# Hansard-T/FHE-Linformer

Measured on AMD Instinct MI355X. Metric: encrypted Linformer-d128 forward ms/sample, lower is better.
Workload: dtype u64

## Files before the change

fhe-linformer_amd/csrc/context.cpp:

```cpp
#include "context.h"
#include <hip/hip_runtime.h>
#include <algorithm>
#include <cstdio>
#include <cstdlib>
#include <cstring>
#include <sys/random.h>
#include <time.h>
#include <cxxabi.h>
#include <dlfcn.h>
#include <execinfo.h>

namespace fhelin {

void hip_check(hipError_t e, const char* what) {
    if (e != hipSuccess) throw Error(FHELIN_ERR_HIP, std::string(what) + ": " + hipGetErrorString(e));
}

void* DevicePool::raw_malloc(size_t bytes) {
    if (backend_.malloc_fn) return backend_.malloc_fn(bytes);
    void* p = nullptr;
    if (hipMalloc(&p, bytes) != hipSuccess) {
        (void)hipGetLastError();
        return nullptr;
    }
    return p;
}
void DevicePool::raw_free(void* p) {
    if (backend_.free_fn) backend_.free_fn(p);
    else (void)hipFree(p);
}
DevicePool::~DevicePool() {
    for (auto& ln : lane_) {
        for (auto& pk : ln.parked)
            for (int k = 0; k < pk.n_ev; ++k) (void)hipEventDestroy(pk.ev[k]);
        for (auto& sl : ln.slabs)
            if (sl.base) raw_free(sl.base);
    }
    for (hipEvent_t e : spare_events_) (void)hipEventDestroy(e);
}
size_t DevicePool::slabs() const {
    size_t n = 0;
    for (const auto& ln : lane_)
        for (const auto& sl : ln.slabs) n += sl.base != nullptr;
    return n;
}
size_t DevicePool::free_ranges() const {
    size_t n = 0;
    for (const auto& ln : lane_) n += ln.by_size.size();
    return n;
}
void DevicePool::erase_size_entry(Lane& ln, int slab, size_t off, size_t len) {
    auto r = ln.by_size.equal_range(len);
    for (auto it = r.first; it != r.second; ++it)
        if (it->second.first == slab && it->second.second == off) {
            ln.by_size.erase(it);
            return;
        }
    throw Error(FHELIN_ERR_INTERNAL, "DevicePool: free list out of step");
}
void DevicePool::insert_free(Lane& ln, int slab, size_t off, size_t len) {
    Slab& sl = ln.slabs[slab];
    auto nxt = sl.free_at.lower_bound(off);
    if (nxt != sl.free_at.begin()) {
        auto prv = std::prev(nxt);
        if (prv->first + prv->second == off) {
            off = prv->first;
            len += prv->second;
            erase_size_entry(ln, slab, prv->first, prv->second);
            sl.free_at.erase(prv);
        }
    }
    if (nxt != sl.free_at.end() && off + len == nxt->first) {
        len += nxt->second;
        erase_size_entry(ln, slab, nxt->first, nxt->second);
        sl.free_at.erase(nxt);
    }
    sl.free_at[off] = len;
    ln.by_size.emplace(len, std::make_pair(slab, off));
}
bool DevicePool::grow(Lane& ln, size_t bytes) {
    size_t want = std::max(bytes, std::min(SLAB_MAX, std::max(SLAB_MIN, reserved_)));
    want = (want + (size_t(2) << 20) - 1) & ~((size_t(2) << 20) - 1);
    timespec t0, t1;
    clock_gettime(CLOCK_MONOTONIC, &t0);
    void* p = raw_malloc(want);
// ... 149 lines not shown
        for (int i = 0; i < 8; ++i) p.seed_bytes[i] = (uint8_t)(p.seed >> (8 * i));
    } else {
        size_t got = 0;
        while (got < sizeof p.seed_bytes) {
            const ssize_t n = getrandom(p.seed_bytes + got, sizeof p.seed_bytes - got, 0);
            if (n <= 0) throw Error(FHELIN_ERR_INTERNAL, "getrandom failed: no entropy for key generation");
            got += (size_t)n;
        }
    }
    p.have_seed_bytes = true;
}

static Params resolve_params(Params p) {
    resolve_seed(p);
    if (p.n_p < 0 && p.n_q >= 1 && p.dnum >= 1 && p.special_bits >= 1) {
        const int a = (p.n_q + p.dnum - 1) / p.dnum;
        const int first = p.first_bits + (std::min(a, p.n_q) - 1) * p.scale_bits;
        const int other = p.n_q > a ? std::min(a, p.n_q - a) * p.scale_bits : 0;
        p.n_p = (std::max(first, other) + p.special_bits - 1) / p.special_bits;
    }
    return p;
}

Context::Context(const Params& p_in) : prm(resolve_params(p_in)) {
    const Params& p = prm;
    if (p.log_n < 12 || p.log_n > 17) throw Error(FHELIN_ERR_ARG, "log_n must be in [12,17]");
    if (p.n_q < 1 || p.n_q > 64 || p.n_p < 0 || p.n_p > 16) throw Error(FHELIN_ERR_ARG, "bad limb counts");
    if (p.dnum < 1) throw Error(FHELIN_ERR_ARG, "dnum must be >= 1");
    if (p.first_bits > 60 || p.scale_bits > 60 || p.special_bits > 60) throw Error(FHELIN_ERR_ARG, "primes must be <= 60 bits");
    if (p.first_bits < 20 || p.scale_bits < 20 || (p.n_p > 0 && p.special_bits < 20)) throw Error(FHELIN_ERR_ARG, "primes must be >= 20 bits");
    if (p.log_slots < 1 || p.log_slots > p.log_n - 1) throw Error(FHELIN_ERR_ARG, "log_slots out of range");
    N = 1 << p.log_n;
    L = p.n_q - 1;
    K = p.n_p;
    alpha = (p.n_q + p.dnum - 1) / p.dnum;
    if (alpha > 16) throw Error(FHELIN_ERR_ARG, "digit size > 16 limbs not supported");
    if ((p.n_q + alpha - 1) / alpha > 16) throw Error(FHELIN_ERR_ARG, "more than 16 key-switching digits not supported");
    try {
        chain = make_prime_chain(p.log_n, p.n_q, p.first_bits, p.scale_bits, p.n_p, p.special_bits);
    } catch (const std::exception& e) {
        throw Error(FHELIN_ERR_ARG, std::string("prime chain: ") + e.what());
    }
    moduli = chain.q;
    moduli.insert(moduli.end(), chain.p.begin(), chain.p.end());
    for (u64 q : moduli) {
        barrett.push_back(h_barrett(q));
        tw.push_back(make_twiddles(q, p.log_n));
    }
    sf_real.assign(p.n_q + 1, 0.0L);
    sf_real[0] = (long double)chain.q[L];
    for (int k = 0; k < L; ++k) sf_real[k + 1] = sf_real[k] * sf_real[k] / (long double)chain.q[L - k];

    if (p.device < 0) return;

    int ndev = 0;
    if (hipGetDeviceCount(&ndev) != hipSuccess || ndev <= 0)
        throw Error(FHELIN_ERR_NO_DEVICE, "no HIP device visible: the fhe-linformer_amd engine has no CPU fallback");
    if (p.device >= ndev) throw Error(FHELIN_ERR_ARG, "device index out of range");
    hip_check(hipSetDevice(p.device), "hipSetDevice");
    hip_check(hipStreamCreateWithFlags(&stream, hipStreamNonBlocking), "hipStreamCreate");
    main_stream = stream;
    own_stream = true;
    {
        int want = 2;
        if (const char* e = std::getenv("FHELIN_LANES")) want = std::atoi(e);
        n_lanes = std::max(0, std::min(want, DevicePool::MAX_LANES - 1));
        for (int k = 1; k <= n_lanes; ++k) {
            hip_check(hipStreamCreateWithFlags(&lane_stream[k], hipStreamNonBlocking), "hipStreamCreate(lane)");
            hip_check(hipEventCreateWithFlags(&lane_event[k], hipEventDisableTiming), "hipEventCreate(lane)");
        }
        hip_check(hipEventCreateWithFlags(&fork_event, hipEventDisableTiming), "hipEventCreate(fork)");
        pool.lane_stream[0] = main_stream;
        for (int k = 1; k <= n_lanes; ++k) pool.lane_stream[k] = lane_stream[k];
        pool.have_streams = true;
        if (const char* e = std::getenv("FHELIN_ASYNC")) async_lanes = std::atoi(e) != 0;
        if (const char* e = std::getenv("FHELIN_FUSE_MODDOWN")) fuse_moddown = std::atoi(e) != 0;
        if (const char* e = std::getenv("FHELIN_FUSE_FINISH")) fuse_finish = std::atoi(e) != 0;
        if (const char* e = std::getenv("FHELIN_HOST_ENCODE")) host_encode = std::atoi(e) != 0;
        if (const char* e = std::getenv("FHELIN_FUSE_GATHER")) fuse_gather = std::atoi(e) != 0;
        if (const char* e = std::getenv("FHELIN_FUSE_LIFT")) fuse_lift = std::atoi(e) != 0;
        if (const char* e = std::getenv("FHELIN_LDS_DIGITS")) lds_digits = std::atoi(e) != 0;
        if (const char* e = std::getenv("FHELIN_NTT_TRACE")) trace_small_ntt = std::atoi(e);
        if (const char* e = std::getenv("FHELIN_HOST_WAITS")) trace_waits = std::atoi(e) != 0;
    }
    hip_check(hipEventCreate(&ev_start), "hipEventCreate");
    stage_words = (size_t)2 << p.log_n;
    for (int i = 0; i < STAGE_SLOTS; ++i) {
        hip_check(hipHostMalloc(reinterpret_cast<void**>(&stage_buf[i]), stage_words * sizeof(u64), hipHostMallocDefault), "hipHostMalloc(stage)");
        hip_check(hipEventCreateWithFlags(&stage_ev[i], hipEventDisableTiming), "hipEventCreate(stage)");
    }
    hip_check(hipHostMalloc(reinterpret_cast<void**>(&small_buf), (size_t)SMALL_SLOTS * SMALL_WORDS * sizeof(u64), hipHostMallocDefault), "hipHostMalloc(stage, small)");
    for (int i = 0; i < SMALL_SLOTS; ++i) hip_check(hipEventCreateWithFlags(&small_ev[i], hipEventDisableTiming), "hipEventCreate(stage, small)");
    hip_check(hipEventCreate(&ev_stop), "hipEventCreate");
    has_device = true;

    const int nl = (int)moduli.size();
    {
        std::vector<u64> bar(2 * nl), ninv(8 * nl, 0);
        for (int i = 0; i < nl; ++i) {
            bar[2 * i] = barrett[i].r0;
            bar[2 * i + 1] = barrett[i].r1;
            ninv[8 * i] = tw[i].n_inv;
            ninv[8 * i + 1] = tw[i].n_inv_s;
            ninv[8 * i + 2] = tw[i].w1_n_inv;
            ninv[8 * i + 3] = tw[i].w1_n_inv_s;
            int bits = 0;
            while (bits < 64 && (moduli[i] >> bits)) ++bits;
            if (bits >= 12 && bits <= 60) {
                ninv[8 * i + 4] = (u64)(bits - 10);
                ninv[8 * i + 5] = (u64)((((u128)1) << (bits + 22)) / moduli[i]);
            }
        }
        dt.log_n = p.log_n;
        dt.n_limbs = nl;
        dt.moduli = upload_table(moduli);
        dt.barrett = upload_table(bar);
        {
            std::vector<u64> qi(nl);
            for (int i = 0; i < nl; ++i) {
                u64 x = moduli[i];
                for (int it = 0; it < 6; ++it) x *= 2 - moduli[i] * x;
                qi[i] = x;
            }
            dt.qinv = upload_table(qi);
            std::vector<u64> mr(2 * (size_t)nl);
            for (int i = 0; i < nl; ++i) {
                mr[2 * i] = mont_r(moduli[i]);
                mr[2 * i + 1] = h_shoup(mr[2 * i], moduli[i]);
            }
            dt.mont = upload_table(mr);
        }
        dt.ninv = upload_table(ninv);
        std::vector<u64> f((size_t)nl * 2 * N), g((size_t)nl * 2 * N);
        for (int i = 0; i < nl; ++i) {
            std::memcpy(&f[(size_t)i * 2 * N], tw[i].fwd.data(), sizeof(u64) * 2 * N);
            std::memcpy(&g[(size_t)i * 2 * N], tw[i].inv.data(), sizeof(u64) * 2 * N);
        }
        dt.tw_fwd = upload_table(f);
        dt.tw_inv = upload_table(g);
        const size_t tiles = N >> 12;
        const size_t per_limb = tiles * 15 * 256 * 2;
        for (int dir = 0; dir < 2; ++dir) {
            const std::vector<u64>& src = dir ? g : f;
            std::vector<u64> r((size_t)nl * per_limb);
            for (int i = 0; i < nl; ++i)
                for (size_t T = 0; T < tiles; ++T)
                    for (int kb = 0; kb < 4; ++kb)
                        for (int j = 0; j < (8 >> kb); ++j)
                            for (size_t tau = 0; tau < 256; ++tau) {
                                const size_t idx = (N >> (kb + 1)) + ((((T << 8) | tau)) << (3 - kb)) + j;
                                const size_t s_ = (size_t)(8 >> kb) - 1 + j;
                                const size_t o = (size_t)i * per_limb + ((T * 15 + s_) * 256 + tau) * 2;
                                r[o] = src[(size_t)i * 2 * N + 2 * idx];
                                r[o + 1] = src[(size_t)i * 2 * N + 2 * idx + 1];
                            }
            (dir ? dt.tw_rows_inv : dt.tw_rows_fwd) = upload_table(r);
        }
    }
    {
        std::vector<u64> phatinv(2 * std::max(K, 1)), phatmod((size_t)std::max(K, 1) * (L + 1)), pinv(2 * (L + 1));
        for (int j = 0; j < K; ++j) {
            u64 pj = chain.p[j];
            u64 hat = prod_mod(chain.p, j, pj);
            u64 inv = h_invmod(hat, pj);
            phatinv[2 * j] = inv;
            phatinv[2 * j + 1] = h_shoup(inv, pj);
// ... 275 lines not shown
```

fhe-linformer_amd/csrc/context.h:

```cpp
#pragma once
#include <cstdint>
#include <map>
#include <memory>
#include <stdexcept>
#include <string>
#include <unordered_map>
#include <vector>
#include <hip/hip_runtime_api.h>
#include "../../include/fhelin.h"
#include "hostmath.h"
#include "kernels.h"

namespace fhelin {

struct Params {
    int log_n = 16;
    int n_q = 24;
    int first_bits = 55;
    int scale_bits = 52;
    int n_p = 6;
    int special_bits = 60;
    int dnum = 4;
    int log_slots = 14;
    int hamming = 192;
// ... 94 lines not shown
    int L = 0;
    int K = 0;
    int alpha = 0;
    PrimeChain chain;
    std::vector<u64> moduli;
    std::vector<Barrett> barrett;
    std::vector<TwiddleTable> tw;
    std::vector<long double> sf_real;

    bool has_device = false;
    hipStream_t stream = nullptr;
    hipStream_t main_stream = nullptr;
    bool own_stream = false;
    int n_lanes = 0;
    hipStream_t lane_stream[DevicePool::MAX_LANES] = {};
    hipEvent_t lane_event[DevicePool::MAX_LANES] = {};
    hipEvent_t fork_event = nullptr;
    bool async_lanes = true;
    int async_rr = 0;
    u64 lane_seq[DevicePool::MAX_LANES] = {};
    std::vector<std::pair<u64, std::shared_ptr<void>>> lane_hold[DevicePool::MAX_LANES];
    void release_holds(int lane, u64 up_to_seq);
    void fork_lanes();
    void join_lanes();
    struct LaneScope {
        Context& c;
        LaneScope(Context& ctx, int k) : c(ctx) {
            c.stream = c.lane_stream[k];
            c.pool.cur_lane = k;
        }
        ~LaneScope() {
            c.stream = c.main_stream;
            c.pool.cur_lane = 0;
        }
    };
    DevicePool pool;
    DeviceTables dt{};
    std::vector<void*> table_allocs;
    hipEvent_t ev_start = nullptr, ev_stop = nullptr;

    static constexpr int STAGE_SLOTS = 64;
    u64* stage_buf[STAGE_SLOTS] = {};
    hipEvent_t stage_ev[STAGE_SLOTS] = {};
    bool stage_used[STAGE_SLOTS] = {};
    int stage_next = 0;
    size_t stage_words = 0;
    static constexpr int SMALL_SLOTS = 256;
    static constexpr size_t SMALL_WORDS = 8192;
    u64* small_buf = nullptr;
    hipEvent_t small_ev[SMALL_SLOTS] = {};
    bool small_used[SMALL_SLOTS] = {};
    int small_next = 0;
    void upload_async(u64* dst, const u64* src, size_t words);

    const u64* d_phatinv = nullptr;
    const u64* d_phatmod = nullptr;
    const u64* d_pinv = nullptr;
    const u64* d_pmod = nullptr;
    const u64* d_qlinv = nullptr;
    const u64* d_qlmod = nullptr;
    std::vector<LevelTables> lvl;
    std::map<u64, const u32*> automorph_maps;

    explicit Context(const Params& p);
    ~Context();
    Context(const Context&) = delete;
    Context& operator=(const Context&) = delete;

    void require_device() const;
    template <class T> T* dalloc(size_t count) { return static_cast<T*>(pool.alloc(count * sizeof(T))); }
    template <class T> const T* upload_table(const std::vector<T>& v);
    int limb_id_q(int i) const { return i; }
    int limb_id_p(int j) const { return L + 1 + j; }
    int digits_at(int ell) const { return (ell + alpha - 1) / alpha; }
    u64 galois_element(int rot_index) const;
    const u32* automorph_map(u64 galois);
    const u32* automorph_inverse_of(const u32* map);
    std::map<const u32*, const u32*> automorph_inverse;
    bool fuse_finish = true;
    bool fuse_moddown = false;
    bool host_encode = false;
    bool fuse_gather = true;
    bool fuse_lift = true;
    bool lds_digits = true;
    struct FftDev {
        const u32* rot = nullptr;
        const double* ksi = nullptr;
    };
    std::map<int, FftDev> fft_dev;
    void sync();
    void ntt(const LimbBatch& b, bool inverse, int active = -1) {
        stats.limb_ntt += (u64)(active >= 0 ? active : b.nvec);
        if (trace_small_ntt && b.nvec <= trace_small_ntt) note_small_ntt(b.nvec);
        launch_ntt(dt, b, inverse, stream);
    }
    bool trace_waits = false;
    std::map<std::string, std::pair<u64, u64>> wait_sites;
    void note_wait(const char* site, u64 ns) {
        auto& e = wait_sites[site];
        e.first += 1;
        e.second += ns;
    }
    int trace_small_ntt = 0;
    std::map<std::string, std::pair<u64, u64>> small_ntt_sites;
    void note_small_ntt(int nvec);
    void ntt_epilogue(const LimbBatch& b, const NttEpilogue& ep) {
        stats.limb_ntt += (u64)b.nvec;
        if (trace_small_ntt && b.nvec <= trace_small_ntt) note_small_ntt(b.nvec);
        launch_ntt_epilogue(dt, b, ep, stream);
    }
};

}
```

fhe-linformer_amd/csrc/kernels.h:

```cpp
#pragma once
#include <cstddef>
#include <cstdint>
#include <hip/hip_runtime_api.h>
#include "modarith.h"

namespace fhelin {

struct LimbBatch {
    u64* data;
    int nvec;
    const int* limb_tab;
    int limb_first;
    int limb_count;
    const u64* src = nullptr;
    int tab_len = 0;
    int src_group = 0;
    size_t src_group_stride = 0;
    int src_group2 = 0;
    size_t src_group2_stride = 0;
    bool lazy_out = false;
    const u64* lift_qlm = nullptr;
    int lift_limb = -1;
};

struct DeviceTables {
    int log_n;
    int n_limbs;
    const u64* moduli;
    const u64* barrett;
    const u64* qinv;
    const u64* mont;
    const u64* tw_fwd;
    const u64* tw_inv;
    const u64* tw_rows_fwd;
    const u64* tw_rows_inv;
    const u64* ninv;
};

struct NttEpilogue {
    static constexpr int MAX_ROWS = 16;
    const u64* acc = nullptr;
    size_t acc_poly_stride = 0;
    u64* out = nullptr;
    size_t out_stride = 0;
    const u64* w = nullptr;
    int ell = 0;
    const u64* add0 = nullptr;
    const u64* add1 = nullptr;
    const u64* post = nullptr;
    size_t add_stride = 0, post_stride = 0;
    const u32* invmap = nullptr;
    int per_row = 0;
    const u32* invmap_row[MAX_ROWS] = {};
};

void launch_ntt(const DeviceTables& t, const LimbBatch& b, bool inverse, hipStream_t s);
void launch_ntt_epilogue(const DeviceTables& t, const LimbBatch& b, const NttEpilogue& ep, hipStream_t s);


}
```

fhe-linformer_amd/csrc/kernels_ntt.hip:

```cpp
#include <hip/hip_runtime.h>
#include <algorithm>
#include <cstdlib>
#include "kernels.h"

namespace fhelin {

namespace {

struct NttArgs {
    u64* data;
    const u64* src;
    const u64* tw;
    const u64* tw_rows;
    const u64* moduli;
    const u64* ninv;
    const int* limb_tab;
    int tab_len;
    int limb_first;
    int limb_count;
    int log_n;
    int nvec;
    int period;
    int lazy_out;
    int src_group;
    size_t src_group_stride;
    int src_group2;
    size_t src_group2_stride;
    const u64* lift_qlm;
    int lift_limb;
    int vec0;
};

__device__ __forceinline__ size_t src_offset(const NttArgs& a, int vec, int log_n) {
    if (a.src_group > 0) {
        const int g = vec / a.src_group;
        const size_t in = (size_t)(vec % a.src_group) << log_n;
        if (a.src_group2 > 0) return (size_t)(g / a.src_group2) * a.src_group2_stride + (size_t)(g % a.src_group2) * a.src_group_stride + in;
        return (size_t)g * a.src_group_stride + in;
    }
    return (size_t)vec << log_n;
}

constexpr int TILE = 4096;
constexpr int LDS_WORDS = TILE + TILE / 16;

__device__ __forceinline__ int tile_index(int tau, int k, int p) {
    return ((tau >> p) << (p + 4)) | (k << p) | (tau & ((1 << p) - 1));
}
__device__ __forceinline__ int lds_slot(int e) { return e + (e >> 4); }

__device__ __forceinline__ int limb_of(const NttArgs& a, int vec) {
    return a.limb_tab ? a.limb_tab[a.tab_len ? vec % a.tab_len : vec] : a.limb_first + (vec % a.limb_count);
}

typedef u64 u64x2 __attribute__((ext_vector_type(2)));

struct LimbConst {
    u64 q;
    u64 nq;
    u64 q5;
    u32 sh;
    u32 rr;
};

struct RoundTw {
    u64x2 t[15];
};
template <int KB_LO, int KB_HI>
__device__ __forceinline__ void load_round_tw(RoundTw& r, const u64x2* __restrict__ tw, int log_n, int gbase, int hi) {
#pragma unroll
    for (int kb = KB_LO; kb < KB_HI; ++kb) {
        const int m = 1 << (log_n - (gbase + kb) - 1);
        const int tbase = m + (hi << (3 - kb));
#pragma unroll
        for (int j = 0; j < (8 >> kb); ++j) r.t[(8 >> kb) - 1 + j] = tw[tbase + j];
    }
}

__device__ __forceinline__ void load_round_tw_rows(RoundTw& r, const u64x2* __restrict__ trows, int tau) {
#pragma unroll
    for (int s = 0; s < 15; ++s) r.t[s] = trows[s * 256 + tau];
}

template <int KB, bool LAZY>
__device__ __forceinline__ void fwd_stage(u64 (&x)[16], const RoundTw& tw, const LimbConst& c) {
#pragma unroll
    for (int k0 = 0; k0 < 16; ++k0) {
        if (k0 & (1 << KB)) continue;
        const int k1 = k0 | (1 << KB);
        const u64x2 w = tw.t[(8 >> KB) - 1 + (k0 >> (KB + 1))];
        const u64 X = LAZY ? x[k0] : csub_mask(x[k0], c.q5);
#if defined(FHELIN_BFLY15)
        const u64 T = mul_shoup_lazy5(x[k1], w.x, w.y, c.nq);
        x[k0] = X + T;
        x[k1] = X + c.q5 - T;
#else
        const u64 A = mul_shoup_lazy5_add(x[k1], w.x, w.y, c.nq, X);
        x[k0] = A;
        x[k1] = shl1_add(X, c.q5) - A;
#endif
    }
}
template <int KB_LO, int KB_HI, bool LAZY>
__device__ __forceinline__ void fwd_round(u64 (&x)[16], const RoundTw& tw, const LimbConst& c) {
    if constexpr (KB_LO < KB_HI) {
        fwd_stage<KB_HI - 1, LAZY>(x, tw, c);
        fwd_round<KB_LO, KB_HI - 1, LAZY>(x, tw, c);
    }
}

constexpr int lazy_coef(int s, int c0) { return s == 0 ? c0 : 5 << (s - 1); }

template <int KB, bool FINAL, bool LAZY, int S, int C0>
__device__ __forceinline__ void inv_stage(u64 (&x)[16], const RoundTw& tw, const LimbConst& c, const u64* __restrict__ ninv) {
    const u64 B = c.q * (u64)lazy_coef(S, C0);
    if constexpr (FINAL) {
        const u64 ni = ninv[0], nis = ninv[1], wn = ninv[2], wns = ninv[3];
#pragma unroll
        for (int k0 = 0; k0 < 16; ++k0) {
            if (k0 & (1 << KB)) continue;
            const int k1 = k0 | (1 << KB);
            const u64 X = x[k0], Y = x[k1];
            if (LAZY) {
                x[k0] = csub_mask(reduce_lazy_2q(mul_shoup_lazy5(X + Y, ni, nis, c.nq), c.q, c.sh, c.rr), c.q);
                x[k1] = csub_mask(reduce_lazy_2q(mul_shoup_lazy5(X + B - Y, wn, wns, c.nq), c.q, c.sh, c.rr), c.q);
            } else {
                x[k0] = csub_mask(reduce_lazy_2q(mul_shoup_lazy5(X + Y, ni, nis, c.nq), c.q, c.sh, c.rr), c.q);
                x[k1] = csub_mask(reduce_lazy_2q(mul_shoup_lazy5(X + c.q5 - Y, wn, wns, c.nq), c.q, c.sh, c.rr), c.q);
            }
        }
    } else {
#pragma unroll
        for (int k0 = 0; k0 < 16; ++k0) {
            if (k0 & (1 << KB)) continue;
            const int k1 = k0 | (1 << KB);
            const u64x2 w = tw.t[(8 >> KB) - 1 + (k0 >> (KB + 1))];
            const u64 X = x[k0], Y = x[k1];
            if (LAZY) {
                x[k0] = X + Y;
                x[k1] = mul_shoup_lazy5(X + B - Y, w.x, w.y, c.nq);
            } else {
                x[k0] = csub_mask(X + Y, c.q5);
                x[k1] = mul_shoup_lazy5(X + c.q5 - Y, w.x, w.y, c.nq);
            }
        }
    }
}
template <int KB_LO, int KB_HI, bool LAST, bool LAZY, int S0 = 0, int C0 = 1>
__device__ __forceinline__ void inv_round(u64 (&x)[16], const RoundTw& tw, const LimbConst& c, const u64* __restrict__ ninv) {
    if constexpr (KB_LO < KB_HI) {
        inv_stage<KB_LO, (LAST && KB_LO == KB_HI - 1), LAZY, S0, C0>(x, tw, c, ninv);
        inv_round<KB_LO + 1, KB_HI, LAST, LAZY, S0 + 1, C0>(x, tw, c, ninv);
    }
}

__device__ __forceinline__ void exchange(u64 (&x)[16], u64* lds, int tau, int p_from, int p_to, bool sync_first) {
    if (sync_first) __syncthreads();
#pragma unroll
    for (int k = 0; k < 16; ++k) lds[lds_slot(tile_index(tau, k, p_from))] = x[k];
    __syncthreads();
#pragma unroll
    for (int k = 0; k < 16; ++k) x[k] = lds[lds_slot(tile_index(tau, k, p_to))];
}

__device__ __forceinline__ LimbConst limb_const(const NttArgs& a, int limb) {
    LimbConst c;
    c.q = a.moduli[limb];
    c.nq = 0 - c.q;
    c.q5 = 5 * c.q;
    c.sh = (u32)a.ninv[8 * limb + 4];
    c.rr = (u32)a.ninv[8 * limb + 5];
    return c;
}
#if defined(FHELIN_NTT_FORCE_PATH)
template <bool INVERSE> __device__ __forceinline__ bool lazy_prime(u64) { return FHELIN_NTT_FORCE_PATH; }
#else
template <bool INVERSE> __device__ __forceinline__ bool lazy_prime(u64 q) { return q < (1ull << (INVERSE ? 53 : 57)); }
#endif

template <int A, bool INVERSE, bool LAZY, bool LIFT>
__device__ __forceinline__ void cols_body(const NttArgs& a, u64* lds, int vec, int tile, int limb, const LimbConst& c) {
    constexpr int LOGCW = 12 - A;
    constexpr int CW = 1 << LOGCW;
    constexpr int LOGN = A + 8;
    constexpr int NFULL = A / 4;
    constexpr int REM = A % 4;
    const u64x2* tw = reinterpret_cast<const u64x2*>(a.tw) + ((size_t)limb << LOGN);
    u64* base = a.data + ((size_t)vec << LOGN) + tile * CW;
    const u64* sbase = (LIFT ? a.src + ((size_t)(vec / a.limb_count) << LOGN) : a.src + src_offset(a, vec, LOGN)) + tile * CW;
    const int tau = threadIdx.x;
    u64 x[16];

    auto goff = [](int e) { return ((e >> LOGCW) << 8) | (e & (CW - 1)); };

    if (!INVERSE) {
        constexpr int P0 = LOGCW + A - 4;
#pragma unroll
        for (int k = 0; k < 16; ++k) x[k] = sbase[goff(tile_index(tau, k, P0))];
        if constexpr (LIFT) {
            const u64 half = a.moduli[a.lift_limb] >> 1, qlm = a.lift_qlm[limb];
#pragma unroll
            for (int k = 0; k < 16; ++k) {
                const u64 r = csub_mask(x[k], c.q);
                x[k] = x[k] > half ? sub_mod(r, qlm, c.q) : r;
            }
        }
        RoundTw rt, rn;
        load_round_tw<0, 4>(rt, tw, LOGN, 8 + P0 - LOGCW, tau >> P0);
        fwd_round<0, 4, LAZY>(x, rt, c);
        int p_prev = P0;
        if constexpr (NFULL >= 2) {
            constexpr int P1 = LOGCW + A - 8;
            load_round_tw<0, 4>(rn, tw, LOGN, 8 + P1 - LOGCW, tau >> P1);
            exchange(x, lds, tau, p_prev, P1, false);
            fwd_round<0, 4, LAZY>(x, rn, c);
            p_prev = P1;
        }
        if constexpr (REM > 0) {
            constexpr int PR = LOGCW;
            load_round_tw<0, REM>(rt, tw, LOGN, 8, tau >> PR);
            exchange(x, lds, tau, p_prev, PR, NFULL >= 2);
            fwd_round<0, REM, LAZY>(x, rt, c);
            p_prev = PR;
        }
        constexpr int PL = REM > 0 ? LOGCW : (NFULL >= 2 ? LOGCW + A - 8 : P0);
        (void)p_prev;
#pragma unroll
        for (int k = 0; k < 16; ++k) base[goff(tile_index(tau, k, PL))] = x[k];
    } else {
        const u64* ninv = a.ninv + 8 * limb;
        constexpr int P0 = LOGCW;
#pragma unroll
        for (int k = 0; k < 16; ++k) x[k] = sbase[goff(tile_index(tau, k, P0))];
        RoundTw rt, rn;
        load_round_tw<0, 4>(rt, tw, LOGN, 8, tau >> P0);
        inv_round<0, 4, (NFULL == 1 && REM == 0), LAZY, 0, 2>(x, rt, c, ninv);
        int p_prev = P0;
        if constexpr (NFULL >= 2) {
            constexpr int P1 = LOGCW + 4;
            load_round_tw<0, 4>(rn, tw, LOGN, 8 + 4, tau >> P1);
            exchange(x, lds, tau, p_prev, P1, false);
            inv_round<0, 4, (REM == 0), LAZY, 4, 2>(x, rn, c, ninv);
            p_prev = P1;
        }
        if constexpr (REM > 0) {
            constexpr int PR = 8;
            load_round_tw<4 - REM, 4>(rt, tw, LOGN, 8 + PR - LOGCW, tau >> PR);
            exchange(x, lds, tau, p_prev, PR, NFULL >= 2);
            inv_round<4 - REM, 4, true, LAZY, 4 * NFULL, 2>(x, rt, c, ninv);
            p_prev = PR;
        }
        constexpr int PL = REM > 0 ? 8 : (NFULL >= 2 ? LOGCW + 4 : P0);
        (void)p_prev;
#pragma unroll
        for (int k = 0; k < 16; ++k) base[goff(tile_index(tau, k, PL))] = x[k];
    }
}

template <int A, bool INVERSE, bool LIFT = false>
__global__ __launch_bounds__(256) __attribute__((amdgpu_waves_per_eu(LIFT ? 3 : 4))) void ntt_cols_kernel(NttArgs a) {
    constexpr int LOGTILES = A - 4;
    __shared__ u64 lds[LDS_WORDS];
    const int vec = a.vec0 + (blockIdx.x >> LOGTILES);
    const int tile = blockIdx.x & ((1 << LOGTILES) - 1);
    const int limb = limb_of(a, vec);
    if (limb < 0) return;
    const LimbConst c = limb_const(a, limb);
    if (lazy_prime<INVERSE>(c.q))
        cols_body<A, INVERSE, true, LIFT>(a, lds, vec, tile, limb, c);
    else
        cols_body<A, INVERSE, false, LIFT>(a, lds, vec, tile, limb, c);
}

template <bool INVERSE, bool LAZY, bool EPI>
__device__ __forceinline__ void rows_body(const NttArgs& a, u64* lds, int vec, int tile, int limb, const LimbConst& c,
                                          const NttEpilogue* ep) {
    const int log_n = a.log_n;
    const u64x2* tw = reinterpret_cast<const u64x2*>(a.tw) + ((size_t)limb << log_n);
    const u64x2* trows = reinterpret_cast<const u64x2*>(a.tw_rows) + (((size_t)limb << (log_n - 12)) + tile) * (15 * 256);
    u64* base = a.data + ((size_t)vec << log_n) + ((size_t)tile << 12);
    const u64* sbase = a.src + src_offset(a, vec, log_n) + ((size_t)tile << 12);
    const int tau = threadIdx.x;
    u64 x[16];

    if (!INVERSE) {
#pragma unroll
        for (int k = 0; k < 16; ++k) x[k] = sbase[tile_index(tau, k, 4)];
        RoundTw rt, rn;
        load_round_tw<0, 4>(rt, tw, log_n, 4, (tile << 4) | (tau >> 4));
        fwd_round<0, 4, LAZY>(x, rt, c);
        load_round_tw_rows(rn, trows, tau);
        exchange(x, lds, tau, 4, 0, false);
        fwd_round<0, 4, LAZY>(x, rn, c);
        [[maybe_unused]] u64 av[16];
        [[maybe_unused]] int ell = 0, t = 0, poly = 0;
        if constexpr (EPI) {
            ell = ep->ell;
            t = vec % ell;
            poly = vec / ell;
            const u64* acc = ep->acc + (size_t)poly * ep->acc_poly_stride + ((size_t)t << log_n) + ((size_t)tile << 12);
#pragma unroll
            for (int k = 0; k < 16; ++k) av[k] = acc[tile_index(tau, k, 8)];
        }
        if constexpr (EPI) {
#pragma unroll
            for (int k = 0; k < 16; ++k) x[k] = reduce_lazy_2q(x[k], c.q, c.sh, c.rr);
        } else if (!(LAZY && a.lazy_out && c.q < (1ull << 53))) {
#pragma unroll
            for (int k = 0; k < 16; ++k)
                x[k] = csub_mask(reduce_lazy_2q(x[k], c.q, c.sh, c.rr), c.q);
        }
#if defined(FHELIN_ROWS_DIRECT_STORE)
        if constexpr (!EPI) {
#pragma unroll
            for (int k = 0; k < 16; k += 2) {
                u64x2 v;
                v.x = x[k];
                v.y = x[k + 1];
                reinterpret_cast<u64x2*>(base + 16 * tau)[k >> 1] = v;
            }
            return;
        }
#endif
        exchange(x, lds, tau, 0, 8, true);
        if constexpr (EPI) {
            const int bi = poly >> 1, comp = poly & 1;
            const size_t n = (size_t)1 << log_n;
            const u64 w = ep->w[2 * t], ws = ep->w[2 * t + 1];
            const u64 q2 = 2 * c.q;
#pragma unroll
            for (int k = 0; k < 16; ++k) x[k] = mul_shoup(av[k] + q2 - x[k], w, ws, c.q);
            const u64* add = comp == 0 ? ep->add0 : ep->add1;
            if (add) {
                add += (size_t)bi * ep->add_stride + (size_t)t * n + ((size_t)tile << 12);
#pragma unroll
                for (int k = 0; k < 16; ++k) x[k] = add_mod(x[k], add[tile_index(tau, k, 8)], c.q);
            }
            const size_t row_off = (size_t)(comp * ell + t) * n;
            const u64* post = ep->post ? ep->post + (size_t)bi * ep->post_stride + row_off : nullptr;
            u64* out = ep->out + (size_t)bi * ep->out_stride + row_off;
            const u32* im = ep->per_row ? ep->invmap_row[bi] : ep->invmap;
            if (im) {
#pragma unroll
                for (int k = 0; k < 16; ++k) {
                    const size_t j = im[((size_t)tile << 12) + tile_index(tau, k, 8)];
                    u64 r = x[k];
                    if (post) r = add_mod(r, post[j], c.q);
                    out[j] = r;
                }
            } else {
                out += (size_t)tile << 12;
                if (post) {
                    post += (size_t)tile << 12;
#pragma unroll
                    for (int k = 0; k < 16; ++k) x[k] = add_mod(x[k], post[tile_index(tau, k, 8)], c.q);
                }
#pragma unroll
                for (int k = 0; k < 16; ++k) out[tile_index(tau, k, 8)] = x[k];
            }
        } else {
#pragma unroll
            for (int k = 0; k < 16; ++k) base[tile_index(tau, k, 8)] = x[k];
        }
    } else {
#pragma unroll
        for (int k = 0; k < 16; ++k) x[k] = sbase[tile_index(tau, k, 8)];
        RoundTw rt, rn;
        load_round_tw_rows(rt, trows, tau);
        exchange(x, lds, tau, 8, 0, false);
        inv_round<0, 4, false, LAZY, 0, 1>(x, rt, c, nullptr);
        load_round_tw<0, 4>(rn, tw, log_n, 4, (tile << 4) | (tau >> 4));
        exchange(x, lds, tau, 0, 4, true);
        inv_round<0, 4, false, LAZY, 4, 1>(x, rn, c, nullptr);
        if (LAZY) {
#pragma unroll
            for (int k = 0; k < 16; ++k) x[k] = reduce_lazy_2q(x[k], c.q, c.sh, c.rr);
        }
#pragma unroll
        for (int k = 0; k < 16; ++k) base[tile_index(tau, k, 4)] = x[k];
    }
}

template <bool INVERSE, bool EPI = false>
__global__ __launch_bounds__(256) __attribute__((amdgpu_waves_per_eu(4))) void ntt_rows_kernel(NttArgs a, NttEpilogue ep) {
    __shared__ u64 lds[LDS_WORDS];
    const int logtiles = a.log_n - 12;
    int lid = blockIdx.x;
    const int nblk = gridDim.x;
    if ((nblk & 7) == 0) lid = (lid & 7) * (nblk >> 3) + (lid >> 3);
    int vec, tile;
    if (a.period > 0) {
        const int nper = a.nvec / a.period;
        const int rep = lid % nper, r = lid / nper;
        tile = r & ((1 << logtiles) - 1);
        vec = a.vec0 + rep * a.period + (r >> logtiles);
    } else {
        vec = a.vec0 + (lid >> logtiles);
        tile = lid & ((1 << logtiles) - 1);
    }
    const int limb = limb_of(a, vec);
    if (limb < 0) return;
    const LimbConst c = limb_const(a, limb);
    if (lazy_prime<INVERSE>(c.q))
        rows_body<INVERSE, true, EPI>(a, lds, vec, tile, limb, c, &ep);
    else
        rows_body<INVERSE, false, EPI>(a, lds, vec, tile, limb, c, &ep);
}

template <int A>
void launch_cols(const NttArgs& a, bool inverse, int blocks, hipStream_t s) {
    if (inverse)
        hipLaunchKernelGGL((ntt_cols_kernel<A, true>), dim3(blocks), dim3(256), 0, s, a);
    else if (a.lift_qlm)
        hipLaunchKernelGGL((ntt_cols_kernel<A, false, true>), dim3(blocks), dim3(256), 0, s, a);
    else
        hipLaunchKernelGGL((ntt_cols_kernel<A, false>), dim3(blocks), dim3(256), 0, s, a);
}

}

static void launch_ntt_impl(const DeviceTables& t, const LimbBatch& b, bool inverse, const NttEpilogue* ep, hipStream_t s);

void launch_ntt(const DeviceTables& t, const LimbBatch& b, bool inverse, hipStream_t s) { launch_ntt_impl(t, b, inverse, nullptr, s); }
void launch_ntt_epilogue(const DeviceTables& t, const LimbBatch& b, const NttEpilogue& ep, hipStream_t s) {
    launch_ntt_impl(t, b, false, &ep, s);
}

static void launch_ntt_impl(const DeviceTables& t, const LimbBatch& b, bool inverse, const NttEpilogue* ep, hipStream_t s) {
    if (b.nvec <= 0) return;
    NttArgs a;
    a.data = b.data;
    a.src = b.src ? b.src : b.data;
    a.src_group = b.src ? b.src_group : 0;
    a.src_group_stride = b.src_group_stride;
    a.src_group2 = (b.src && b.src_group > 0) ? b.src_group2 : 0;
    a.src_group2_stride = b.src_group2_stride;
    a.lazy_out = (!inverse && b.lazy_out) ? 1 : 0;
    a.lift_qlm = (!inverse && b.src && b.lift_limb >= 0) ? b.lift_qlm : nullptr;
    a.lift_limb = b.lift_limb;
    a.tw = inverse ? t.tw_inv : t.tw_fwd;
    a.tw_rows = inverse ? t.tw_rows_inv : t.tw_rows_fwd;
    a.moduli = t.moduli;
    a.ninv = t.ninv;
    a.limb_tab = b.limb_tab;
    a.tab_len = b.tab_len;
    a.limb_first = b.limb_first;
    a.limb_count = b.limb_count > 0 ? b.limb_count : 1;
    a.log_n = t.log_n;
    a.nvec = b.nvec;
    const int per = b.limb_tab ? b.tab_len : a.limb_count;
    a.period = (per > 0 && per < b.nvec && b.nvec % per == 0) ? per : 0;
    const int A = t.log_n - 8;
    a.vec0 = 0;
    static const int chunk_mb = [] {
        const char* e = std::getenv("FHELIN_NTT_CHUNK_MB");
        return e ? std::atoi(e) : 0;
    }();
    int chunk = b.nvec;
    if (chunk_mb > 0 && !ep) {
        const size_t vec_bytes = (size_t)8 << t.log_n;
        const int want = (int)std::max<size_t>(1, ((size_t)chunk_mb << 20) / vec_bytes);
        if (b.nvec > want + want / 2) {
            const int per = a.period > 0 ? a.period : 1;
            chunk = std::max(per, want / per * per);
        }
    }
    const int nvec_all = b.nvec, period_all = a.period;
    const u64* src_all = a.src;
    const int sg = a.src_group, sg2 = a.src_group2;
    for (int v0 = 0; v0 < nvec_all; v0 += chunk) {
        a.vec0 = v0;
        a.nvec = std::min(chunk, nvec_all - v0);
        a.period = (period_all > 0 && a.nvec % period_all == 0 && a.nvec > period_all) ? period_all : 0;
        a.src = src_all;
        a.src_group = sg;
        a.src_group2 = sg2;
        const int blocks = a.nvec << (t.log_n - 12);
        auto cols = [&]() {
            switch (A) {
                case 4: launch_cols<4>(a, inverse, blocks, s); break;
                case 5: launch_cols<5>(a, inverse, blocks, s); break;
                case 6: launch_cols<6>(a, inverse, blocks, s); break;
                case 7: launch_cols<7>(a, inverse, blocks, s); break;
                case 8: launch_cols<8>(a, inverse, blocks, s); break;
                case 9: launch_cols<9>(a, inverse, blocks, s); break;
                default: break;
            }
        };
        if (!inverse) {
            cols();
            a.src = a.data;
            a.src_group = 0;
            a.src_group2 = 0;
            if (ep)
                hipLaunchKernelGGL((ntt_rows_kernel<false, true>), dim3(blocks), dim3(256), 0, s, a, *ep);
            else
                hipLaunchKernelGGL((ntt_rows_kernel<false, false>), dim3(blocks), dim3(256), 0, s, a, NttEpilogue());
        } else {
            hipLaunchKernelGGL((ntt_rows_kernel<true, false>), dim3(blocks), dim3(256), 0, s, a, NttEpilogue());
            a.src = a.data;
            a.src_group = 0;
            a.src_group2 = 0;
            cols();
        }
    }
}

}
```

Measured before the change: 239.4.

## Add narrow NTT kernels with more threads per tile for small batches

Adds NTT column and row kernel variants that hold 8 (or 4) elements per thread instead of 16, launched with 512 or 1024 threads per 4096-element tile. They are selected when the launch has fewer blocks than a CU-count-based threshold, so small NTT batches can fill the GPU with more threads. The cost is extra LDS exchange rounds and barriers per tile, plus more template instantiations. An environment variable can force the narrow path on or off.

Result: no change. 238.2 (median of 6 runs) (-0.5%).

```diff
diff --git a/fhe-linformer_amd/csrc/context.cpp b/fhe-linformer_amd/csrc/context.cpp
--- a/fhe-linformer_amd/csrc/context.cpp
+++ b/fhe-linformer_amd/csrc/context.cpp
@@ -1,6 +1,7 @@
 #include "context.h"
 #include <hip/hip_runtime.h>
 #include <algorithm>
+#include <climits>
 #include <cstdio>
 #include <cstdlib>
 #include <cstring>
@@ -316,6 +317,17 @@
         if (const char* e = std::getenv("FHELIN_LDS_DIGITS")) lds_digits = std::atoi(e) != 0;
         if (const char* e = std::getenv("FHELIN_NTT_TRACE")) trace_small_ntt = std::atoi(e);
         if (const char* e = std::getenv("FHELIN_HOST_WAITS")) trace_waits = std::atoi(e) != 0;
+        int cus = 0;
+        hip_check(hipDeviceGetAttribute(&cus, hipDeviceAttributeMultiprocessorCount, p.device), "hipDeviceGetAttribute(CUs)");
+        dt.ntt_narrow_below = NTT_NARROW_BLOCKS_PER_CU * std::max(cus, 1);
+        if (const char* e = std::getenv("FHELIN_NTT_NARROW")) {
+            if (!std::strcmp(e, "0"))
+                dt.ntt_narrow_below = 0;
+            else if (!std::strcmp(e, "1"))
+                dt.ntt_narrow_below = INT_MAX;
+            else if (std::strcmp(e, "auto"))
+                throw Error(FHELIN_ERR_ARG, "FHELIN_NTT_NARROW must be auto, 0 or 1");
+        }
     }
     hip_check(hipEventCreate(&ev_start), "hipEventCreate");
     stage_words = (size_t)2 << p.log_n;
diff --git a/fhe-linformer_amd/csrc/context.h b/fhe-linformer_amd/csrc/context.h
--- a/fhe-linformer_amd/csrc/context.h
+++ b/fhe-linformer_amd/csrc/context.h
@@ -200,6 +200,7 @@
     bool host_encode = false;
     bool fuse_gather = true;
     bool fuse_lift = true;
+    static constexpr int NTT_NARROW_BLOCKS_PER_CU = 6;
     bool lds_digits = true;
     struct FftDev {
         const u32* rot = nullptr;
diff --git a/fhe-linformer_amd/csrc/kernels.h b/fhe-linformer_amd/csrc/kernels.h
--- a/fhe-linformer_amd/csrc/kernels.h
+++ b/fhe-linformer_amd/csrc/kernels.h
@@ -35,6 +35,7 @@
     const u64* tw_rows_fwd;
     const u64* tw_rows_inv;
     const u64* ninv;
+    int ntt_narrow_below;
 };
 
 struct NttEpilogue {
diff --git a/fhe-linformer_amd/csrc/kernels_ntt.hip b/fhe-linformer_amd/csrc/kernels_ntt.hip
--- a/fhe-linformer_amd/csrc/kernels_ntt.hip
+++ b/fhe-linformer_amd/csrc/kernels_ntt.hip
@@ -44,9 +44,11 @@
 constexpr int TILE = 4096;
 constexpr int LDS_WORDS = TILE + TILE / 16;
 
+template <int W = 4>
 __device__ __forceinline__ int tile_index(int tau, int k, int p) {
-    return ((tau >> p) << (p + 4)) | (k << p) | (tau & ((1 << p) - 1));
-}
+    return ((tau >> p) << (p + W)) | (k << p) | (tau & ((1 << p) - 1));
+}
+constexpr int log2i(int r) { return r <= 1 ? 0 : 1 + log2i(r / 2); }
 __device__ __forceinline__ int lds_slot(int e) { return e + (e >> 4); }
 
 __device__ __forceinline__ int limb_of(const NttArgs& a, int vec) {
@@ -63,9 +65,11 @@
     u32 rr;
 };
 
-struct RoundTw {
-    u64x2 t[15];
+template <int R>
+struct RoundTwR {
+    u64x2 t[R - 1];
 };
+using RoundTw = RoundTwR<16>;
 template <int KB_LO, int KB_HI>
 __device__ __forceinline__ void load_round_tw(RoundTw& r, const u64x2* __restrict__ tw, int log_n, int gbase, int hi) {
 #pragma unroll
@@ -82,13 +86,13 @@
     for (int s = 0; s < 15; ++s) r.t[s] = trows[s * 256 + tau];
 }
 
-template <int KB, bool LAZY>
-__device__ __forceinline__ void fwd_stage(u64 (&x)[16], const RoundTw& tw, const LimbConst& c) {
-#pragma unroll
-    for (int k0 = 0; k0 < 16; ++k0) {
+template <int KB, bool LAZY, int R>
+__device__ __forceinline__ void fwd_stage(u64 (&x)[R], const RoundTwR<R>& tw, const LimbConst& c) {
+#pragma unroll
+    for (int k0 = 0; k0 < R; ++k0) {
         if (k0 & (1 << KB)) continue;
         const int k1 = k0 | (1 << KB);
-        const u64x2 w = tw.t[(8 >> KB) - 1 + (k0 >> (KB + 1))];
+        const u64x2 w = tw.t[((R / 2) >> KB) - 1 + (k0 >> (KB + 1))];
         const u64 X = LAZY ? x[k0] : csub_mask(x[k0], c.q5);
 #if defined(FHELIN_BFLY15)
         const u64 T = mul_shoup_lazy5(x[k1], w.x, w.y, c.nq);
@@ -101,8 +105,8 @@
 #endif
     }
 }
-template <int KB_LO, int KB_HI, bool LAZY>
-__device__ __forceinline__ void fwd_round(u64 (&x)[16], const RoundTw& tw, const LimbConst& c) {
+template <int KB_LO, int KB_HI, bool LAZY, int R>
+__device__ __forceinline__ void fwd_round(u64 (&x)[R], const RoundTwR<R>& tw, const LimbConst& c) {
     if constexpr (KB_LO < KB_HI) {
         fwd_stage<KB_HI - 1, LAZY>(x, tw, c);
         fwd_round<KB_LO, KB_HI - 1, LAZY>(x, tw, c);
@@ -111,13 +115,13 @@
 
 constexpr int lazy_coef(int s, int c0) { return s == 0 ? c0 : 5 << (s - 1); }
 
-template <int KB, bool FINAL, bool LAZY, int S, int C0>
-__device__ __forceinline__ void inv_stage(u64 (&x)[16], const RoundTw& tw, const LimbConst& c, const u64* __restrict__ ninv) {
+template <int KB, bool FINAL, bool LAZY, int S, int C0, int R>
+__device__ __forceinline__ void inv_stage(u64 (&x)[R], const RoundTwR<R>& tw, const LimbConst& c, const u64* __restrict__ ninv) {
     const u64 B = c.q * (u64)lazy_coef(S, C0);
     if constexpr (FINAL) {
         const u64 ni = ninv[0], nis = ninv[1], wn = ninv[2], wns = ninv[3];
 #pragma unroll
-        for (int k0 = 0; k0 < 16; ++k0) {
+        for (int k0 = 0; k0 < R; ++k0) {
             if (k0 & (1 << KB)) continue;
             const int k1 = k0 | (1 << KB);
             const u64 X = x[k0], Y = x[k1];
@@ -131,10 +135,10 @@
         }
     } else {
 #pragma unroll
-        for (int k0 = 0; k0 < 16; ++k0) {
+        for (int k0 = 0; k0 < R; ++k0) {
             if (k0 & (1 << KB)) continue;
             const int k1 = k0 | (1 << KB);
-            const u64x2 w = tw.t[(8 >> KB) - 1 + (k0 >> (KB + 1))];
+            const u64x2 w = tw.t[((R / 2) >> KB) - 1 + (k0 >> (KB + 1))];
             const u64 X = x[k0], Y = x[k1];
             if (LAZY) {
                 x[k0] = X + Y;
@@ -146,21 +150,23 @@
         }
     }
 }
-template <int KB_LO, int KB_HI, bool LAST, bool LAZY, int S0 = 0, int C0 = 1>
-__device__ __forceinline__ void inv_round(u64 (&x)[16], const RoundTw& tw, const LimbConst& c, const u64* __restrict__ ninv) {
+template <int KB_LO, int KB_HI, bool LAST, bool LAZY, int S0 = 0, int C0 = 1, int R>
+__device__ __forceinline__ void inv_round(u64 (&x)[R], const RoundTwR<R>& tw, const LimbConst& c, const u64* __restrict__ ninv) {
     if constexpr (KB_LO < KB_HI) {
         inv_stage<KB_LO, (LAST && KB_LO == KB_HI - 1), LAZY, S0, C0>(x, tw, c, ninv);
         inv_round<KB_LO + 1, KB_HI, LAST, LAZY, S0 + 1, C0>(x, tw, c, ninv);
     }
 }
 
-__device__ __forceinline__ void exchange(u64 (&x)[16], u64* lds, int tau, int p_from, int p_to, bool sync_first) {
+template <int R>
+__device__ __forceinline__ void exchange(u64 (&x)[R], u64* lds, int tau, int p_from, int p_to, bool sync_first) {
+    constexpr int W = log2i(R);
     if (sync_first) __syncthreads();
 #pragma unroll
-    for (int k = 0; k < 16; ++k) lds[lds_slot(tile_index(tau, k, p_from))] = x[k];
+    for (int k = 0; k < R; ++k) lds[lds_slot(tile_index<W>(tau, k, p_from))] = x[k];
     __syncthreads();
 #pragma unroll
-    for (int k = 0; k < 16; ++k) x[k] = lds[lds_slot(tile_index(tau, k, p_to))];
+    for (int k = 0; k < R; ++k) x[k] = lds[lds_slot(tile_index<W>(tau, k, p_to))];
 }
 
 __device__ __forceinline__ LimbConst limb_const(const NttArgs& a, int limb) {
@@ -177,6 +183,66 @@
 #else
 template <bool INVERSE> __device__ __forceinline__ bool lazy_prime(u64 q) { return q < (1ull << (INVERSE ? 53 : 57)); }
 #endif
+
+template <int R>
+__device__ __forceinline__ void lift_centred(u64 (&x)[R], const NttArgs& a, int limb, const LimbConst& c) {
+    const u64 half = a.moduli[a.lift_limb] >> 1, qlm = a.lift_qlm[limb];
+#pragma unroll
+    for (int k = 0; k < R; ++k) {
+        const u64 r = csub_mask(x[k], c.q);
+        x[k] = x[k] > half ? sub_mod(r, qlm, c.q) : r;
+    }
+}
+
+#ifndef FHELIN_NTT_NARROW_RPT
+#define FHELIN_NTT_NARROW_RPT 8
+#endif
+constexpr int NARROW_W = log2i(FHELIN_NTT_NARROW_RPT);
+static_assert(NARROW_W == 2 || NARROW_W == 3, "FHELIN_NTT_NARROW_RPT must be 4 or 8");
+
+constexpr int fwd_win(int lo, int hi, int w) { return hi - w > lo ? hi - w : lo; }
+constexpr int inv_win(int lo, int hi, int w) { return lo + w <= hi ? lo : hi - w; }
+constexpr int inv_top(int lo, int hi, int w) { return lo + w < hi ? lo + w : hi; }
+
+template <int P, int KB_LO, int KB_HI, int R, class F>
+__device__ __forceinline__ void load_round_tw_by(RoundTwR<R>& r, int tau, const F& twf) {
+    constexpr int W = log2i(R);
+#pragma unroll
+    for (int kb = KB_LO; kb < KB_HI; ++kb) {
+#pragma unroll
+        for (int j = 0; j < ((R / 2) >> kb); ++j) r.t[((R / 2) >> kb) - 1 + j] = twf(P + kb, tile_index<W>(tau, j << (kb + 1), P));
+    }
+}
+
+template <int LO, int HI, bool LAZY, int R, class F>
+__device__ __forceinline__ void fwd_rounds(u64 (&x)[R], const RoundTwR<R>& rt, u64* lds, int tau, const LimbConst& c, const F& twf,
+                                           bool sync_first) {
+    constexpr int W = log2i(R);
+    constexpr int P = fwd_win(LO, HI, W);
+    fwd_round<0, HI - P, LAZY>(x, rt, c);
+    if constexpr (P > LO) {
+        constexpr int PN = fwd_win(LO, P, W);
+        RoundTwR<R> rn;
+        load_round_tw_by<PN, 0, P - PN>(rn, tau, twf);
+        exchange(x, lds, tau, P, PN, sync_first);
+        fwd_rounds<LO, P, LAZY>(x, rn, lds, tau, c, twf, true);
+    }
+}
+
+template <int LO, int HI, bool LAST, bool LAZY, int S0, int C0, int R, class F>
+__device__ __forceinline__ void inv_rounds(u64 (&x)[R], const RoundTwR<R>& rt, u64* lds, int tau, const LimbConst& c,
+                                           const u64* __restrict__ ninv, const F& twf, bool sync_first) {
+    constexpr int W = log2i(R);
+    constexpr int P = inv_win(LO, HI, W), TOP = inv_top(LO, HI, W);
+    inv_round<LO - P, TOP - P, LAST && TOP == HI, LAZY, S0, C0>(x, rt, c, ninv);
+    if constexpr (TOP < HI) {
+        constexpr int PN = inv_win(TOP, HI, W), TN = inv_top(TOP, HI, W);
+        RoundTwR<R> rn;
+        load_round_tw_by<PN, TOP - PN, TN - PN>(rn, tau, twf);
+        exchange(x, lds, tau, P, PN, sync_first);
+        inv_rounds<TOP, HI, LAST, LAZY, S0 + TOP - LO, C0>(x, rn, lds, tau, c, ninv, twf, true);
+    }
+}
 
 template <int A, bool INVERSE, bool LAZY, bool LIFT>
 __device__ __forceinline__ void cols_body(const NttArgs& a, u64* lds, int vec, int tile, int limb, const LimbConst& c) {
@@ -197,14 +263,7 @@
         constexpr int P0 = LOGCW + A - 4;
 #pragma unroll
         for (int k = 0; k < 16; ++k) x[k] = sbase[goff(tile_index(tau, k, P0))];
-        if constexpr (LIFT) {
-            const u64 half = a.moduli[a.lift_limb] >> 1, qlm = a.lift_qlm[limb];
-#pragma unroll
-            for (int k = 0; k < 16; ++k) {
-                const u64 r = csub_mask(x[k], c.q);
-                x[k] = x[k] > half ? sub_mod(r, qlm, c.q) : r;
-            }
-        }
+        if constexpr (LIFT) lift_centred(x, a, limb, c);
         RoundTw rt, rn;
         load_round_tw<0, 4>(rt, tw, LOGN, 8 + P0 - LOGCW, tau >> P0);
         fwd_round<0, 4, LAZY>(x, rt, c);
@@ -257,8 +316,43 @@
     }
 }
 
-template <int A, bool INVERSE, bool LIFT = false>
-__global__ __launch_bounds__(256) __attribute__((amdgpu_waves_per_eu(LIFT ? 3 : 4))) void ntt_cols_kernel(NttArgs a) {
+template <int A, bool INVERSE, bool LAZY, bool LIFT, int W>
+__device__ __forceinline__ void cols_body_narrow(const NttArgs& a, u64* lds, int vec, int tile, int limb, const LimbConst& c) {
+    constexpr int R = 1 << W;
+    constexpr int LOGCW = 12 - A;
+    constexpr int CW = 1 << LOGCW;
+    constexpr int LOGN = A + 8;
+    const u64x2* tw = reinterpret_cast<const u64x2*>(a.tw) + ((size_t)limb << LOGN);
+    u64* base = a.data + ((size_t)vec << LOGN) + tile * CW;
+    const u64* sbase = (LIFT ? a.src + ((size_t)(vec / a.limb_count) << LOGN) : a.src + src_offset(a, vec, LOGN)) + tile * CW;
+    const int tau = threadIdx.x;
+    u64 x[R];
+    auto goff = [](int e) { return ((e >> LOGCW) << 8) | (e & (CW - 1)); };
+    auto twf = [&](int b, int e) { return tw[(1 << (11 - b)) + (e >> (b + 1))]; };
+    RoundTwR<R> rt;
+    if (!INVERSE) {
+        constexpr int P0 = fwd_win(LOGCW, 12, W);
+#pragma unroll
+        for (int k = 0; k < R; ++k) x[k] = sbase[goff(tile_index<W>(tau, k, P0))];
+        if constexpr (LIFT) lift_centred(x, a, limb, c);
+        load_round_tw_by<P0, 0, 12 - P0>(rt, tau, twf);
+        fwd_rounds<LOGCW, 12, LAZY>(x, rt, lds, tau, c, twf, false);
+#pragma unroll
+        for (int k = 0; k < R; ++k) base[goff(tile_index<W>(tau, k, LOGCW))] = x[k];
+    } else {
+        const u64* ninv = a.ninv + 8 * limb;
+        constexpr int P0 = inv_win(LOGCW, 12, W), T0 = inv_top(LOGCW, 12, W);
+#pragma unroll
+        for (int k = 0; k < R; ++k) x[k] = sbase[goff(tile_index<W>(tau, k, P0))];
+        load_round_tw_by<P0, LOGCW - P0, T0 - P0>(rt, tau, twf);
+        inv_rounds<LOGCW, 12, true, LAZY, 0, 2>(x, rt, lds, tau, c, ninv, twf, false);
+#pragma unroll
+        for (int k = 0; k < R; ++k) base[goff(tile_index<W>(tau, k, 12 - W))] = x[k];
+    }
+}
+
+template <int A, bool INVERSE, bool LIFT = false, int W = 4>
+__global__ __launch_bounds__(4096 >> W) __attribute__((amdgpu_waves_per_eu(W == 4 && LIFT ? 3 : 4))) void ntt_cols_kernel(NttArgs a) {
     constexpr int LOGTILES = A - 4;
     __shared__ u64 lds[LDS_WORDS];
     const int vec = a.vec0 + (blockIdx.x >> LOGTILES);
@@ -266,10 +360,82 @@
     const int limb = limb_of(a, vec);
     if (limb < 0) return;
     const LimbConst c = limb_const(a, limb);
-    if (lazy_prime<INVERSE>(c.q))
-        cols_body<A, INVERSE, true, LIFT>(a, lds, vec, tile, limb, c);
-    else
-        cols_body<A, INVERSE, false, LIFT>(a, lds, vec, tile, limb, c);
+    if constexpr (W == 4) {
+        if (lazy_prime<INVERSE>(c.q))
+            cols_body<A, INVERSE, true, LIFT>(a, lds, vec, tile, limb, c);
+        else
+            cols_body<A, INVERSE, false, LIFT>(a, lds, vec, tile, limb, c);
+    } else {
+        if (lazy_prime<INVERSE>(c.q))
+            cols_body_narrow<A, INVERSE, true, LIFT, W>(a, lds, vec, tile, limb, c);
+        else
+            cols_body_narrow<A, INVERSE, false, LIFT, W>(a, lds, vec, tile, limb, c);
+    }
+}
+
+template <bool LAZY, bool EPI, int R>
+__device__ __forceinline__ void rows_fwd_finish(const NttArgs& a, u64* lds, u64* base, int vec, int tile, const LimbConst& c,
+                                                const NttEpilogue* ep, u64 (&x)[R], int tau) {
+    constexpr int W = log2i(R);
+    const int log_n = a.log_n;
+    [[maybe_unused]] u64 av[R];
+    [[maybe_unused]] int ell = 0, t = 0, poly = 0;
+    if constexpr (EPI) {
+        ell = ep->ell;
+        t = vec % ell;
+        poly = vec / ell;
+        const u64* acc = ep->acc + (size_t)poly * ep->acc_poly_stride + ((size_t)t << log_n) + ((size_t)tile << 12);
+#pragma unroll
+        for (int k = 0; k < R; ++k) av[k] = acc[tile_index<W>(tau, k, 8)];
+    }
+    if constexpr (EPI) {
+#pragma unroll
+        for (int k = 0; k < R; ++k) x[k] = reduce_lazy_2q(x[k], c.q, c.sh, c.rr);
+    } else if (!(LAZY && a.lazy_out && c.q < (1ull << 53))) {
+#pragma unroll
+        for (int k = 0; k < R; ++k)
+            x[k] = csub_mask(reduce_lazy_2q(x[k], c.q, c.sh, c.rr), c.q);
+    }
+    exchange(x, lds, tau, 0, 8, true);
+    if constexpr (EPI) {
+        const int bi = poly >> 1, comp = poly & 1;
+        const size_t n = (size_t)1 << log_n;
+        const u64 w = ep->w[2 * t], ws = ep->w[2 * t + 1];
+        const u64 q2 = 2 * c.q;
+#pragma unroll
+        for (int k = 0; k < R; ++k) x[k] = mul_shoup(av[k] + q2 - x[k], w, ws, c.q);
+        const u64* add = comp == 0 ? ep->add0 : ep->add1;
+        if (add) {
+            add += (size_t)bi * ep->add_stride + (size_t)t * n + ((size_t)tile << 12);
+#pragma unroll
+            for (int k = 0; k < R; ++k) x[k] = add_mod(x[k], add[tile_index<W>(tau, k, 8)], c.q);
+        }
+        const size_t row_off = (size_t)(comp * ell + t) * n;
+        const u64* post = ep->post ? ep->post + (size_t)bi * ep->post_stride + row_off : nullptr;
+        u64* out = ep->out + (size_t)bi * ep->out_stride + row_off;
+        const u32* im = ep->per_row ? ep->invmap_row[bi] : ep->invmap;
+        if (im) {
+#pragma unroll
+            for (int k = 0; k < R; ++k) {
+                const size_t j = im[((size_t)tile << 12) + tile_index<W>(tau, k, 8)];
+                u64 r = x[k];
+                if (post) r = add_mod(r, post[j], c.q);
+                out[j] = r;
+            }
+        } else {
+            out += (size_t)tile << 12;
+            if (post) {
+                post += (size_t)tile << 12;
+#pragma unroll
+                for (int k = 0; k < R; ++k) x[k] = add_mod(x[k], post[tile_index<W>(tau, k, 8)], c.q);
+            }
+#pragma unroll
+            for (int k = 0; k < R; ++k) out[tile_index<W>(tau, k, 8)] = x[k];
+        }
+    } else {
+#pragma unroll
+        for (int k = 0; k < R; ++k) base[tile_index<W>(tau, k, 8)] = x[k];
+    }
 }
 
 template <bool INVERSE, bool LAZY, bool EPI>
@@ -381,8 +547,47 @@
     }
 }
 
-template <bool INVERSE, bool EPI = false>
-__global__ __launch_bounds__(256) __attribute__((amdgpu_waves_per_eu(4))) void ntt_rows_kernel(NttArgs a, NttEpilogue ep) {
+template <bool INVERSE, bool LAZY, bool EPI, int W>
+__device__ __forceinline__ void rows_body_narrow(const NttArgs& a, u64* lds, int vec, int tile, int limb, const LimbConst& c,
+                                                 const NttEpilogue* ep) {
+    constexpr int R = 1 << W;
+    const int log_n = a.log_n;
+    const u64x2* tw = reinterpret_cast<const u64x2*>(a.tw) + ((size_t)limb << log_n);
+    const u64x2* trows = reinterpret_cast<const u64x2*>(a.tw_rows) + (((size_t)limb << (log_n - 12)) + tile) * (15 * 256);
+    u64* base = a.data + ((size_t)vec << log_n) + ((size_t)tile << 12);
+    const u64* sbase = a.src + src_offset(a, vec, log_n) + ((size_t)tile << 12);
+    const int tau = threadIdx.x;
+    u64 x[R];
+    auto twf = [&](int b, int e) {
+        if (b >= 4) return tw[(1 << (log_n - b - 1)) + (((tile << 12) | e) >> (b + 1))];
+        return trows[((8 >> b) - 1 + ((e & 15) >> (b + 1))) * 256 + (e >> 4)];
+    };
+    RoundTwR<R> rt;
+    if (!INVERSE) {
+        constexpr int P0 = fwd_win(0, 8, W);
+#pragma unroll
+        for (int k = 0; k < R; ++k) x[k] = sbase[tile_index<W>(tau, k, P0)];
+        load_round_tw_by<P0, 0, 8 - P0>(rt, tau, twf);
+        fwd_rounds<0, 8, LAZY>(x, rt, lds, tau, c, twf, false);
+        rows_fwd_finish<LAZY, EPI>(a, lds, base, vec, tile, c, ep, x, tau);
+    } else {
+        constexpr int P0 = inv_win(0, 8, W), T0 = inv_top(0, 8, W);
+#pragma unroll
+        for (int k = 0; k < R; ++k) x[k] = sbase[tile_index<W>(tau, k, 8)];
+        load_round_tw_by<P0, 0, T0 - P0>(rt, tau, twf);
+        exchange(x, lds, tau, 8, P0, false);
+        inv_rounds<0, 8, false, LAZY, 0, 1>(x, rt, lds, tau, c, nullptr, twf, true);
+        if (LAZY) {
+#pragma unroll
+            for (int k = 0; k < R; ++k) x[k] = reduce_lazy_2q(x[k], c.q, c.sh, c.rr);
+        }
+#pragma unroll
+        for (int k = 0; k < R; ++k) base[tile_index<W>(tau, k, 8 - W)] = x[k];
+    }
+}
+
+template <bool INVERSE, bool EPI = false, int W = 4>
+__global__ __launch_bounds__(4096 >> W) __attribute__((amdgpu_waves_per_eu(4))) void ntt_rows_kernel(NttArgs a, NttEpilogue ep) {
     __shared__ u64 lds[LDS_WORDS];
     const int logtiles = a.log_n - 12;
     int lid = blockIdx.x;
@@ -401,20 +606,45 @@
     const int limb = limb_of(a, vec);
     if (limb < 0) return;
     const LimbConst c = limb_const(a, limb);
-    if (lazy_prime<INVERSE>(c.q))
-        rows_body<INVERSE, true, EPI>(a, lds, vec, tile, limb, c, &ep);
-    else
-        rows_body<INVERSE, false, EPI>(a, lds, vec, tile, limb, c, &ep);
-}
-
-template <int A>
+    if constexpr (W == 4) {
+        if (lazy_prime<INVERSE>(c.q))
+            rows_body<INVERSE, true, EPI>(a, lds, vec, tile, limb, c, &ep);
+        else
+            rows_body<INVERSE, false, EPI>(a, lds, vec, tile, limb, c, &ep);
+    } else {
+        if (lazy_prime<INVERSE>(c.q))
+            rows_body_narrow<INVERSE, true, EPI, W>(a, lds, vec, tile, limb, c, &ep);
+        else
+            rows_body_narrow<INVERSE, false, EPI, W>(a, lds, vec, tile, limb, c, &ep);
+    }
+}
+
+template <int A, int W>
 void launch_cols(const NttArgs& a, bool inverse, int blocks, hipStream_t s) {
     if (inverse)
-        hipLaunchKernelGGL((ntt_cols_kernel<A, true>), dim3(blocks), dim3(256), 0, s, a);
+        hipLaunchKernelGGL((ntt_cols_kernel<A, true, false, W>), dim3(blocks), dim3(4096 >> W), 0, s, a);
     else if (a.lift_qlm)
-        hipLaunchKernelGGL((ntt_cols_kernel<A, false, true>), dim3(blocks), dim3(256), 0, s, a);
+        hipLaunchKernelGGL((ntt_cols_kernel<A, false, true, W>), dim3(blocks), dim3(4096 >> W), 0, s, a);
     else
-        hipLaunchKernelGGL((ntt_cols_kernel<A, false>), dim3(blocks), dim3(256), 0, s, a);
+        hipLaunchKernelGGL((ntt_cols_kernel<A, false, false, W>), dim3(blocks), dim3(4096 >> W), 0, s, a);
+}
+template <int A>
+void launch_cols(const NttArgs& a, bool inverse, bool narrow, int blocks, hipStream_t s) {
+    if (narrow)
+        launch_cols<A, NARROW_W>(a, inverse, blocks, s);
+    else
+        launch_cols<A, 4>(a, inverse, blocks, s);
+}
+template <bool INVERSE, bool EPI, int W>
+void launch_rows(const NttArgs& a, const NttEpilogue& ep, int blocks, hipStream_t s) {
+    hipLaunchKernelGGL((ntt_rows_kernel<INVERSE, EPI, W>), dim3(blocks), dim3(4096 >> W), 0, s, a, ep);
+}
+template <bool INVERSE, bool EPI>
+void launch_rows(const NttArgs& a, const NttEpilogue& ep, bool narrow, int blocks, hipStream_t s) {
+    if (narrow)
+        launch_rows<INVERSE, EPI, NARROW_W>(a, ep, blocks, s);
+    else
+        launch_rows<INVERSE, EPI, 4>(a, ep, blocks, s);
 }
 
 }
@@ -476,14 +706,15 @@
         a.src_group = sg;
         a.src_group2 = sg2;
         const int blocks = a.nvec << (t.log_n - 12);
+        const bool narrow = blocks < t.ntt_narrow_below;
         auto cols = [&]() {
             switch (A) {
-                case 4: launch_cols<4>(a, inverse, blocks, s); break;
-                case 5: launch_cols<5>(a, inverse, blocks, s); break;
-                case 6: launch_cols<6>(a, inverse, blocks, s); break;
-                case 7: launch_cols<7>(a, inverse, blocks, s); break;
-                case 8: launch_cols<8>(a, inverse, blocks, s); break;
-                case 9: launch_cols<9>(a, inverse, blocks, s); break;
+                case 4: launch_cols<4>(a, inverse, narrow, blocks, s); break;
+                case 5: launch_cols<5>(a, inverse, narrow, blocks, s); break;
+                case 6: launch_cols<6>(a, inverse, narrow, blocks, s); break;
+                case 7: launch_cols<7>(a, inverse, narrow, blocks, s); break;
+                case 8: launch_cols<8>(a, inverse, narrow, blocks, s); break;
+                case 9: launch_cols<9>(a, inverse, narrow, blocks, s); break;
                 default: break;
             }
         };
@@ -493,11 +724,11 @@
             a.src_group = 0;
             a.src_group2 = 0;
             if (ep)
-                hipLaunchKernelGGL((ntt_rows_kernel<false, true>), dim3(blocks), dim3(256), 0, s, a, *ep);
+                launch_rows<false, true>(a, *ep, narrow, blocks, s);
             else
-                hipLaunchKernelGGL((ntt_rows_kernel<false, false>), dim3(blocks), dim3(256), 0, s, a, NttEpilogue());
+                launch_rows<false, false>(a, NttEpilogue(), narrow, blocks, s);
         } else {
-            hipLaunchKernelGGL((ntt_rows_kernel<true, false>), dim3(blocks), dim3(256), 0, s, a, NttEpilogue());
+            launch_rows<true, false>(a, NttEpilogue(), narrow, blocks, s);
             a.src = a.data;
             a.src_group = 0;
             a.src_group2 = 0;
```
